# Nikhil-Doye/voice-enabled-browser-automation

Measured on AMD Instinct MI355X. Metric: voice-to-intent p50 latency (ms) + ASR RTF; 10s utterance; Llama-3-8B brain, lower is better.
Workload: dtype bf16; 1 GPU; model=whisper-tiny + llama3-8b, global_batch=1, parallelism=dp1, budget_chars=512, hipgraph=True

## Files before the change

### csrc/bindings.cpp

```cpp
#include <mutex>
#include <torch/extension.h>
#include <ATen/hip/impl/HIPStreamMasqueradingAsCUDA.h>
#include <c10/core/DeviceGuard.h>

#include "kernels/vwa_kernels.h"

namespace {

using at::Tensor;

hipStream_t cur_stream(const Tensor& t) {
  return c10::hip::getCurrentHIPStreamMasqueradingAsCUDA(t.device().index()).stream();
}

const uint16_t* bfp(const Tensor& t) { return reinterpret_cast<const uint16_t*>(t.data_ptr()); }
uint16_t* bfp_mut(const Tensor& t) { return reinterpret_cast<uint16_t*>(t.data_ptr()); }
const uint16_t* bfp_opt(const c10::optional<Tensor>& t) { return t.has_value() ? bfp(*t) : nullptr; }

void check_bf16(const Tensor& t, const char* name) {
  TORCH_CHECK(t.is_cuda(), name, " must be a GPU tensor");
  TORCH_CHECK(t.scalar_type() == at::kBFloat16, name, " must be bf16");
}
void check_contig_rows(const Tensor& t, const char* name) {
  TORCH_CHECK(t.dim() == 2, name, " must be 2-D");
// ... 513 lines not shown
  p.ldr = (int)h.stride(0);
}

DecodeAttnParams decode_params(const Tensor& q, const Tensor& k, const Tensor& v, const Tensor& table,
                               int64_t block_size, int64_t sb, int64_t sh, int64_t stok, const Tensor& ctx_lens,
                               const Tensor& seq_ids, int64_t n_q_heads, int64_t n_kv_heads, int64_t head_dim,
                               double scale, int64_t n_splits, const Tensor& part_o, const Tensor& part_ml,
                               const Tensor& counters, const Tensor& out);

std::tuple<Tensor, int64_t> chain_make(Tensor h, Tensor att, Tensor act, Tensor w_o, Tensor w_gu, Tensor w_down,
                                       double eps, c10::optional<Tensor> w_qkv, int64_t n_q_heads, int64_t n_kv_heads,
                                       int64_t head_dim, c10::optional<Tensor> positions, c10::optional<Tensor> slots,
                                       c10::optional<Tensor> rope, c10::optional<Tensor> q_out,
                                       c10::optional<Tensor> k_cache, c10::optional<Tensor> v_cache, Tensor bar,
                                       Tensor work, c10::optional<Tensor> ts, int64_t bar_mode,
                                       c10::optional<Tensor> a_q, c10::optional<Tensor> a_k, c10::optional<Tensor> a_v,
                                       c10::optional<Tensor> a_table, int64_t a_block_size, int64_t a_sb, int64_t a_sh,
                                       int64_t a_st, c10::optional<Tensor> a_ctx, c10::optional<Tensor> a_seq,
                                       double a_scale, int64_t a_n_splits, c10::optional<Tensor> a_part_o,
                                       c10::optional<Tensor> a_part_ml, c10::optional<Tensor> a_counters,
                                       bool w_tiled, c10::optional<Tensor> a_row_table,
                                       c10::optional<Tensor> s_o, c10::optional<Tensor> s_gu,
                                       c10::optional<Tensor> s_down, c10::optional<Tensor> s_qkv, int64_t tp_ar,
                                       c10::optional<Tensor> a_plan, int64_t a_plan_mode) {
  c10::DeviceGuard g(h.device());
  const int64_t M = h.size(0);
  TORCH_CHECK(att.size(0) == M && act.size(0) == M, "row counts differ");
  TORCH_CHECK(act.size(1) * 2 == w_gu.size(0) && w_gu.size(0) % 32 == 0, "act must be [M, gate_up rows / 2]");
  TORCH_CHECK(w_down.size(1) == act.size(1) && w_down.size(0) == h.size(1) && w_o.size(0) == h.size(1),
              "down / o_proj shapes");
  TORCH_CHECK(bar.is_cuda() && bar.scalar_type() == at::kInt && bar.numel() >= 384 && bar.is_contiguous() &&
                  (reinterpret_cast<uintptr_t>(bar.data_ptr()) & 127) == 0,
              "bar must be a 128-byte aligned int32[>=384] on the GPU");
  ChainParams cp{};
  TORCH_CHECK(s_o.has_value() == s_gu.has_value() && s_o.has_value() == s_down.has_value() &&
                  (!w_qkv.has_value() || s_qkv.has_value() == s_o.has_value()),
              "fp8 chain: every phase's weight needs its scales");
  TORCH_CHECK(!s_o.has_value() || w_tiled, "fp8 chain: tiled fp8 weights only");
  cp.ph[0].p = base_params(att, w_o, c10::nullopt, false, eps, s_o, w_tiled);
  cp.ph[0].epi = 1;
  set_resid(cp.ph[0].p, h);
  cp.ph[1].p = base_params(h, w_gu, c10::nullopt, true, eps, s_gu, w_tiled);
  cp.ph[1].epi = 2;
  check_bf16(act, "act");
  TORCH_CHECK(act.stride(1) == 1, "act rows must be contiguous");
  cp.ph[1].p.Y = act.data_ptr();
  cp.ph[1].p.ldy = (int)act.stride(0);
// ... 46 lines not shown
    cp.attn = decode_params(*a_q, *a_k, *a_v, *a_table, a_block_size, a_sb, a_sh, a_st, *a_ctx, *a_seq, n_q_heads,
                            n_kv_heads, head_dim, a_scale, a_n_splits, *a_part_o, *a_part_ml, *a_counters, att);
    TORCH_CHECK(a_n_splits > 1, "attention phase: the in-launch chunk merge needs n_splits > 1");
    cp.attn_g = (int)(n_q_heads / n_kv_heads);
    TORCH_CHECK(a_row_table.has_value(), "attention phase: a_row_table (per-row block tables) is required");
    TORCH_CHECK(a_block_size == 16, "attention phase: 16-token KV blocks (mq_attention.h FINE addressing)");
    {
      const Tensor& rtab = *a_row_table;
      TORCH_CHECK(rtab.is_cuda() && rtab.scalar_type() == at::kInt && rtab.dim() == 2 && rtab.is_contiguous() &&
                      rtab.size(0) >= M && rtab.size(1) <= 128 && rtab.size(1) % 2 == 0,
                  "a_row_table must be int32 [>= rows, <= 128 (even)] contiguous");
      cp.attn.row_table = rtab.data_ptr<int>();
      cp.attn.rt_stride = (int)rtab.size(1);
    }
    if (a_plan_mode) {
      TORCH_CHECK(a_plan_mode == 1 || a_plan_mode == 2, "a_plan_mode: 1 write, 2 read");
      TORCH_CHECK(a_plan.has_value() && a_plan->is_cuda() && a_plan->scalar_type() == at::kInt && a_plan->is_contiguous() &&
                      a_plan->numel() >= (int64_t)chain_grid(h.device().index()) * 16,
                  "a_plan must be int32 [>= grid * 16] on the GPU");
      cp.attn.plan = a_plan->data_ptr<int>();
      cp.attn.plan_mode = (int)a_plan_mode;
    }
  }
  const int lds = vwa_chain_prepare(&cp, chain_grid(h.device().index()));
  if (lds < 0) return {torch::empty({0}, torch::dtype(torch::kUInt8).device(h.device())), 0};
  Tensor host = torch::empty({(int64_t)sizeof(ChainParams)}, torch::dtype(torch::kUInt8));
  std::memcpy(host.data_ptr(), &cp, sizeof(ChainParams));
  return {host.to(h.device()), (int64_t)lds | (cp.n >= 3 && cp.ph[2].xg ? (int64_t)1 << 24 : 0) |
                                    (cp.d_nt2 ? (int64_t)1 << 27 : 0) |
                                    (s_o.has_value() ? (int64_t)1 << 25 : 0) | (cp.o_nt2 ? (int64_t)1 << 26 : 0)};
}

std::tuple<Tensor, int64_t> chain_make_seq(int64_t seq, std::vector<Tensor> X, std::vector<Tensor> W,
                                           std::vector<c10::optional<Tensor>> bias,
                                           std::vector<c10::optional<Tensor>> ln_c, std::vector<Tensor> Y,
                                           std::vector<int64_t> epi, double eps, int64_t n_heads, int64_t head_dim,
                                           c10::optional<Tensor> positions, c10::optional<Tensor> slots,
                                           c10::optional<Tensor> k_cache, c10::optional<Tensor> v_cache, Tensor bar,
                                           Tensor work, int64_t bar_mode, bool w_tiled) {
  const size_t n = X.size();
  TORCH_CHECK(n >= 2 && n <= (size_t)kChainMaxPhases && W.size() == n && bias.size() == n && ln_c.size() == n &&
                  Y.size() == n && epi.size() == n,
              "chain_make_seq: one X/W/bias/ln_c/Y/epi per phase");
  TORCH_CHECK(seq == 1 || seq == 2, "chain_make_seq: seq 1 (Whisper tail) or 2 (Whisper middle)");
  c10::DeviceGuard g(X[0].device());
  TORCH_CHECK(bar.is_cuda() && bar.scalar_type() == at::kInt && bar.numel() >= 384 && bar.is_contiguous() &&
                  (reinterpret_cast<uintptr_t>(bar.data_ptr()) & 127) == 0,
              "bar must be a 128-byte aligned int32[>=384] on the GPU");
// ... 700 lines not shown
  m.def("ar_destroy", &ar_destroy);
  m.doc() = "MI355X (gfx950) HIP kernels for the voice-web-agent inference engine";
  m.def("skinny_gemm", &skinny_gemm, py::arg("x"), py::arg("w"), py::arg("bias"), py::arg("y"), py::arg("epi"),
        py::arg("fuse_rms"), py::arg("eps"), py::arg("residual"), py::arg("w_scale") = py::none(),
        py::arg("ln_c") = py::none(), py::arg("w_tiled") = false, py::arg("col_mask") = py::none(),
        py::arg("col_mask_off") = 0, py::arg("mask_rows") = 1);
  m.def("skinny_gemm_swiglu", &skinny_gemm_swiglu, py::arg("x"), py::arg("w_gu"), py::arg("bias"), py::arg("h"),
        py::arg("fuse_rms"), py::arg("eps"), py::arg("w_scale") = py::none(), py::arg("w_tiled") = false);
  m.def("skinny_gemm_qkv", &skinny_gemm_qkv, py::arg("x"), py::arg("w_qkv"), py::arg("bias"), py::arg("fuse_rms"),
        py::arg("eps"), py::arg("n_q_heads"), py::arg("n_kv_heads"), py::arg("head_dim"), py::arg("use_rope"),
        py::arg("positions"), py::arg("slots"), py::arg("rope"), py::arg("q_out"), py::arg("k_cache"),
        py::arg("v_cache"), py::arg("w_scale") = py::none(), py::arg("ln_c") = py::none(),
        py::arg("w_tiled") = false);
  m.def("chain_make", &chain_make, py::arg("h"), py::arg("att"), py::arg("act"), py::arg("w_o"), py::arg("w_gu"),
        py::arg("w_down"), py::arg("eps"), py::arg("w_qkv"), py::arg("n_q_heads"), py::arg("n_kv_heads"),
        py::arg("head_dim"), py::arg("positions"), py::arg("slots"), py::arg("rope"), py::arg("q_out"),
        py::arg("k_cache"), py::arg("v_cache"), py::arg("bar"), py::arg("work"), py::arg("ts") = py::none(), py::arg("bar_mode") = 1,
        py::arg("a_q") = py::none(), py::arg("a_k") = py::none(), py::arg("a_v") = py::none(),
        py::arg("a_table") = py::none(), py::arg("a_block_size") = 0, py::arg("a_sb") = 0, py::arg("a_sh") = 0,
        py::arg("a_st") = 0, py::arg("a_ctx") = py::none(), py::arg("a_seq") = py::none(), py::arg("a_scale") = 0.0,
        py::arg("a_n_splits") = 0, py::arg("a_part_o") = py::none(), py::arg("a_part_ml") = py::none(),
        py::arg("a_counters") = py::none(), py::arg("w_tiled") = false, py::arg("a_row_table") = py::none(),
        py::arg("s_o") = py::none(), py::arg("s_gu") = py::none(), py::arg("s_down") = py::none(),
        py::arg("s_qkv") = py::none(), py::arg("tp_ar") = 0, py::arg("a_plan") = py::none(), py::arg("a_plan_mode") = 0);
  m.def("set_small_gemm_bytes", &set_small_gemm_bytes);
  m.def("gemm_set_p8", [](int64_t mode) { vwa_gemm_set_p8((int)mode); });
  m.def("skinny_set_x_skew", [](int64_t skew) { vwa_skinny_set_x_skew((int)skew); });
  m.def("gemm_set_split_fill", [](int64_t pct) { vwa_gemm_set_split_fill((int)pct); });
  m.def("chain_make_seq", &chain_make_seq, py::arg("seq"), py::arg("X"), py::arg("W"), py::arg("bias"),
        py::arg("ln_c"), py::arg("Y"), py::arg("epi"), py::arg("eps"), py::arg("n_heads"), py::arg("head_dim"),
        py::arg("positions"), py::arg("slots"), py::arg("k_cache"), py::arg("v_cache"), py::arg("bar"),
        py::arg("work"), py::arg("bar_mode") = 1, py::arg("w_tiled") = false);
  m.def("chain_run", &chain_run, py::arg("desc"), py::arg("n_phases"), py::arg("lds"), py::arg("like"),
        py::arg("attn_g") = 0, py::arg("seq") = 0, py::arg("n_layers") = 1);
  m.def("alloc_uncached_i32", &alloc_uncached_i32);
  m.def("device_cus", [](Tensor like) { return (int64_t)device_cus(like); });
  m.def("wdec_layers", &wdec_layers, py::arg("flat"), py::arg("n_layers"), py::arg("like"));
  m.def("wdec_run", &wdec_run, py::arg("layers"), py::arg("roles"), py::arg("bufs"), py::arg("ints"), py::arg("eps"),
        py::arg("scale"), py::arg("n_prod"), py::arg("ts") = py::none(), py::arg("opt") = 0, py::arg("lm") = py::none(),
        py::arg("emb") = py::none(), py::arg("smp") = py::none(), py::arg("loop_base_block") = 0);
  m.def("decode_advance", &decode_advance);
  m.def("gemm", &gemm, py::arg("x"), py::arg("w"), py::arg("bias"), py::arg("y"), py::arg("epi"),
        py::arg("rstd") = py::none(), py::arg("residual") = py::none(), py::arg("w_tiled") = false,
        py::arg("ws") = py::none(), py::arg("ss_out") = py::none(), py::arg("ss_zero") = py::none(),
        py::arg("ss_in") = py::none(), py::arg("ss_eps") = 1e-5);
  m.def("row_rstd", &row_rstd);
  m.def("gemm_qkv", &gemm_qkv, py::arg("x"), py::arg("sx"), py::arg("w"), py::arg("sw"), py::arg("bias"),
// ... 29 lines not shown
```

### csrc/kernels/skinny_stream.hip

```cpp
#include "common.h"
#include "vwa_kernels.h"
#include "mq_attention.h"

using namespace vwa;

namespace {

enum Epi { EPI_STORE = 0, EPI_RESID = 1, EPI_SWIGLU = 2, EPI_GELU = 3, EPI_QKV = 4 };

constexpr unsigned kOOB = 0xFFFFFFF0u;

VWA_DEVICE uint4 bload(__amdgpu_buffer_rsrc_t r, unsigned off) {
  u32x4 v = __builtin_amdgcn_raw_buffer_load_b128(r, (int)off, 0, 0);
  return make_uint4(v.x, v.y, v.z, v.w);
}
template <int AUX>
VWA_DEVICE uint4 bload_w(__amdgpu_buffer_rsrc_t r, unsigned off) {
  u32x4 v = __builtin_amdgcn_raw_buffer_load_b128(r, (int)off, 0, AUX);
  return make_uint4(v.x, v.y, v.z, v.w);
}
constexpr unsigned kOOB2 = 0x80000000u;
template <int AUX>
VWA_DEVICE uint4 bload_w_so(__amdgpu_buffer_rsrc_t r, unsigned voff, int soff) {
  u32x4 v = __builtin_amdgcn_raw_buffer_load_b128(r, (int)voff, soff, AUX);
// ... 809 lines not shown
  chain_load<S::NT, S::U, WA, R, XG, F8>(ph.p, ph.nb, wr, it, r);
}

template <int NT, int KS>
VWA_DEVICE void tile_publish(int M, float* red, f32x4 (&acc)[NT], float* slot) {
  const int lane = VWA_TX & 63, w = VWA_TX >> 6;
#pragma unroll
  for (int nt = 0; nt < NT; ++nt)
#pragma unroll
    for (int i = 0; i < 4; ++i) red[((w * NT + nt) * 4 + i) * 64 + lane] = acc[nt][i];
  lds_sync();
  for (int o = VWA_TX; o < M * 16 * NT; o += KS * 64) {
    const int m = o / (16 * NT), nn = o % (16 * NT);
    const int nt = nn >> 4, q = nn & 15;
    const int ln = q + 16 * (m >> 2), i = m & 3;
    float v = 0.f;
#pragma unroll
    for (int ww = 0; ww < KS; ++ww) v += red[((ww * NT + nt) * 4 + i) * 64 + ln];
    st_f32<true>(slot + o, v);
  }
  lds_sync();
}

template <int EPI, int KS, int WA, bool XG = false, bool F8 = false, bool W2 = false, int R>
VWA_DEVICE void chain_phase(const ChainParams& cp, int i, uint4 (&X0)[R], uint4 (&X1)[R], char* smem, int pre2,
                            int hs = 0, int wb0 = 0, int wn = 0, bool has0 = true) {
  constexpr int NT = PhaseShape<EPI, KS, XG, F8, W2>::NT, U = PhaseShape<EPI, KS, XG, F8, W2>::U;
  const ChainPhase& ph = cp.ph[i];
  const SkinnyParams& p = ph.p;
  const int nb = ph.nb, M = p.M, K = p.K;
  const int xstride = K + 8;
  u16* xs = reinterpret_cast<u16*>(smem);
  const int xbytes = XG ? 0 : ((M * xstride * 2) + 15) & ~15;
  float* red = reinterpret_cast<float*>(smem + xbytes);
  float* rs = red + KS * NT * 4 * 64;
  float* mu = rs + 16;
  int* s_flag = reinterpret_cast<int*>(rs + 32);
  const float* mus = p.fuse_rms == 2 ? mu : nullptr;
  const int lane = VWA_TX & 63, w = VWA_TX >> 6;
  const int nl = lane & 15, g = lane >> 4;
  const PhaseRange r = chain_range<KS>(ph, wb0, wn);
  const int first_tile = r.u0 / nb;
  const bool xdma = cp.xdma != 0, stager = xdma && w == KS - 1 && !XG;
  auto pst = [&](int k) {
    const int slot = k < 8 ? 22 + 8 * i + k : -1;
    if (cp.ts && VWA_TX == 0 && slot >= 0) *gp(cp.ts + blockIdx.x * kTsStride + slot) = __builtin_amdgcn_s_memrealtime();
  };
  pst(0);
  if constexpr (XG) {
    chain_load_x<U>(p, nb, X0, 0, r);
    if (pre2) chain_load_x<U>(p, nb, X1, 1, r);
  }
  const int k8 = K / 8;
  const __amdgpu_buffer_rsrc_t rx =
      __builtin_amdgcn_make_buffer_rsrc(const_cast<u16*>(p.X), (short)0, (int)((size_t)M * p.ldx * 2), 0x00020000);
  if (stager) {
    const int pieces = K / 512;
    for (int m = 0; m < M; ++m)
      for (int j = 0; j < pieces; ++j)
        __builtin_amdgcn_raw_ptr_buffer_load_lds(
            rx, (__attribute__((address_space(3))) void*)(xs + m * xstride + j * 512), 16,
            (unsigned)(((size_t)m * p.ldx + j * 512) * 2 + lane * 16), 0, 0, 16);
    asm volatile("" ::: "memory");
  }
  const bool xw = xdma && cp.xwait;
  if (xdma && cp.xfirst && !xw) lds_sync();
  auto issue_rest = [&]() {
    if (xdma && !stager && !has0) chain_load<NT, U, WA, R, XG, F8>(p, nb, X0, 0, r);
    if (xdma && !stager && (!pre2 || !has0)) chain_load<NT, U, WA, R, XG, F8>(p, nb, X1, 1, r);
  };
  if (!xw) issue_rest();

  EpiPre pre;
  if (r.n_items > 0 && !xw) epi_values<EPI, NT, true>(p, first_tile, VWA_TX, pre);
  if (stager && xw) {
    asm volatile("s_waitcnt vmcnt(0)" ::: "memory");
  } else if (stager) {
    int nw = 0;
    if (hs < 1) {
      chain_load<NT, U, WA, R, XG, F8>(p, nb, X0, 0, r);
      ++nw;
    }
    if (hs < 2) {
      chain_load<NT, U, WA, R, XG, F8>(p, nb, X1, 1, r);
      ++nw;
    }
    if constexpr (R == 16) {
      if (nw == 2) asm volatile("s_waitcnt vmcnt(32)" ::: "memory");
      else if (nw == 1) asm volatile("s_waitcnt vmcnt(16)" ::: "memory");
      else asm volatile("s_waitcnt vmcnt(0)" ::: "memory");
    } else {
      static_assert(R == 8, "item sizes: 16 or 8 loads");
      if (nw == 2) asm volatile("s_waitcnt vmcnt(16)" ::: "memory");
      else if (nw == 1) asm volatile("s_waitcnt vmcnt(8)" ::: "memory");
      else asm volatile("s_waitcnt vmcnt(0)" ::: "memory");
    }
  } else if (!xdma && !XG) {
    for (int c = VWA_TX; c < M * k8; c += KS * 64) {
      const int m = c / k8, kk = c % k8;
      const u32x4 v = __builtin_amdgcn_raw_buffer_load_b128(rx, (int)(((size_t)m * p.ldx + kk * 8) * 2), 0, 16);
      *reinterpret_cast<uint4*>(xs + m * xstride + kk * 8) = make_uint4(v.x, v.y, v.z, v.w);
    }
  }
  lds_sync();
  pst(1);
  auto issue_xw = [&]() {
    issue_rest();
    if (stager) {
      if (hs < 1) chain_load<NT, U, WA, R, XG, F8>(p, nb, X0, 0, r);
      if (hs < 2) chain_load<NT, U, WA, R, XG, F8>(p, nb, X1, 1, r);
    }
    if (r.n_items > 0) epi_values<EPI, NT, true>(p, first_tile, VWA_TX, pre);
  };
  if (xw && !cp.xw_late) issue_xw();
  for (int m = w; m < 16; m += KS) {
    float sc = 1.f, mean = 0.f;
    if (p.fuse_rms && m < M && !XG) {
      float s = 0.f, s1 = 0.f;
      for (int kk = lane; kk < k8; kk += 64) {
        float f[8];
        unpack8(*reinterpret_cast<const uint4*>(xs + m * xstride + kk * 8), f);
#pragma unroll
        for (int j = 0; j < 8; ++j) {
          s += f[j] * f[j];
          s1 += f[j];
        }
      }
// ... 173 lines not shown
  const int tx = VWA_TX, lane = tx & 63, w = tx >> 6;
  const __amdgpu_buffer_rsrc_t rk = __builtin_amdgcn_make_buffer_rsrc(const_cast<u16*>(a.kv.k), (short)0, 0x7FFFFFF0, 0x00020000);
  const __amdgpu_buffer_rsrc_t rv = __builtin_amdgcn_make_buffer_rsrc(const_cast<u16*>(a.kv.v), (short)0, 0x7FFFFFF0, 0x00020000);
  const __amdgpu_buffer_rsrc_t rt = __builtin_amdgcn_make_buffer_rsrc(const_cast<int*>(a.row_table), (short)0,
                                                                     (r0 + 1) * a.rt_stride * 4, 0x00020000);
  auto* dst = (__attribute__((address_space(3))) void*)(lds + w * kMqStep * 256);
  int blk[4];
#pragma unroll
  for (int i = 0; i < 4; ++i) {
    const int q = w * 64 + lane + 512 * i, key = kbeg + q / 16;
    blk[i] = (int)__builtin_amdgcn_raw_buffer_load_b32(rt, q < nk * 16 ? (r0 * a.rt_stride + key / 16) * 4 : 0x7FFFFFF0,
                                                       0, 0);
  }
#pragma unroll
  for (int i = 0; i < 4; ++i) {
    const int q = w * 64 + lane + 512 * i, key = kbeg + q / 16;
    if (512 * i + w * 64 >= nk * 16) break;
    const long long e = (long long)blk[i] * a.kv.stride_block + (long long)kvh * a.kv.stride_head +
                        (long long)(key & 15) * a.kv.stride_tok;
    const unsigned off = q < nk * 16 ? (unsigned)(e * 2 + (q & 15) * 16) : 0x7FFFFFF0u;
    __builtin_amdgcn_raw_ptr_buffer_load_lds(rk, dst, 16, off, 0, 0, 0);
    __builtin_amdgcn_raw_ptr_buffer_load_lds(rv, dst, 16, off, 0, 0, 0);
  }
}

template <int KS, int SEQ, int NPH, int AG, int WA, bool XG2 = false, bool F8 = false, bool O2 = false, bool D2 = false,
          bool MULTI = false>
__global__ __launch_bounds__(KS * 64) void chain_kernel(const ChainParams* __restrict__ cpp, int n_layers) {
  extern __shared__ __attribute__((aligned(16))) char smem[];
  static_assert(!MULTI || (SEQ == 0 && NPH == 4 && AG > 0 && !XG2), "multi-layer launch: Llama tails with attention");
  const int nwg = (int)gridDim.x;
  unsigned long long* bar = reinterpret_cast<unsigned long long*>(cpp->bar);
  unsigned long long bar_next = chain_base(bar, nwg, cpp->bar_mode);
  const bool tpr = cpp->tp.world > 1;
  const int e0 = tpr ? __hip_atomic_load(gp(cpp->tp.epoch), __ATOMIC_RELAXED, __HIP_MEMORY_SCOPE_AGENT) : 0;
  unsigned long long qkv_base[8] = {};
  const bool qsig = MULTI && cpp->qkv_flags && cpp->bar_mode == 2 && cpp->ph[3].nb == 1 &&
                    cpp->ph[3].p.n_kv_heads <= 8 && cpp->attn_flag;
  if constexpr (MULTI) {
    if (qsig && VWA_TX < 64) {
      const unsigned long long tpg = (unsigned long long)qkv_tiles_per_group(cpp->ph[3].p);
      for (int g = 0; g < cpp->ph[3].p.n_kv_heads; ++g) {
        const unsigned long long v = __hip_atomic_load(gp(&bar[kBarQkv + kBarQkvStride * g]), __ATOMIC_RELAXED, __HIP_MEMORY_SCOPE_AGENT);
        qkv_base[g] = v / tpg * tpg;
      }
    }
  }
  bool pf_prev = false, pf_next = false;
  for (int li = 0; li < (MULTI ? n_layers : 1); ++li) {
  pf_prev = pf_next;
  pf_next = false;
  const ChainParams& cp = cpp[li];
  static_assert(sizeof(ChainParams) <= 25 * 64, "descriptor warm-up covers 25 lines");
  {
    unsigned junk;
    asm("s_load_dword %0, %1, 0x0\n\t""s_load_dword %0, %1, 0x40\n\t""s_load_dword %0, %1, 0x80\n\t""s_load_dword %0, %1, 0xc0\n\t"
        "s_load_dword %0, %1, 0x100\n\t""s_load_dword %0, %1, 0x140\n\t""s_load_dword %0, %1, 0x180\n\t""s_load_dword %0, %1, 0x1c0\n\t"
        "s_load_dword %0, %1, 0x200\n\t""s_load_dword %0, %1, 0x240\n\t""s_load_dword %0, %1, 0x280\n\t""s_load_dword %0, %1, 0x2c0\n\t"
        "s_load_dword %0, %1, 0x300\n\t""s_load_dword %0, %1, 0x340\n\t""s_load_dword %0, %1, 0x380\n\t""s_load_dword %0, %1, 0x3c0\n\t"
        "s_load_dword %0, %1, 0x400\n\t""s_load_dword %0, %1, 0x440\n\t""s_load_dword %0, %1, 0x480\n\t""s_load_dword %0, %1, 0x4c0\n\t""s_load_dword %0, %1, 0x500\n\t"
        "s_load_dword %0, %1, 0x540\n\t""s_load_dword %0, %1, 0x580\n\t""s_load_dword %0, %1, 0x5c0\n\t""s_load_dword %0, %1, 0x600\n\t"
        "s_waitcnt lgkmcnt(0)"
        : "=&s"(junk)
        : "s"(cpp + li));
    if (junk == 0x9e3779b9u) __builtin_amdgcn_s_sleep(1);
  }
  uint4 A[ChainShape<KS, F8>::R] = {}, B[ChainShape<KS, F8>::R] = {};
  unsigned long long gen;
  const int er = e0 + 2 * li;
  int nts = 0;
  auto stamp = [&]() {
    if (cp.ts && VWA_TX == 0) *gp(cp.ts + blockIdx.x * kTsStride + nts) = __builtin_amdgcn_s_memrealtime();
// ... 145 lines not shown
   }
  }
  if constexpr (MULTI) {
    if (li + 1 < n_layers) {
      if (qsig) qkv_signal<KS>(cp.ph[3], bar);
      else gen = chain_arrive(bar, nwg, cp.bar_mode, bar_next);
      const DecodeAttnParams& na = cpp[li + 1].attn;
      int st = 3, ev = 0;
      if (cpp[li + 1].attn_flag && na.plan_mode == 2) {
        const __amdgpu_buffer_rsrc_t r_pl =
            __builtin_amdgcn_make_buffer_rsrc(na.plan, (short)0, ((int)blockIdx.x + 1) * 64, 0x00020000);
        ev = (int)__builtin_amdgcn_raw_buffer_load_b32(r_pl, ((int)blockIdx.x * 16 + (VWA_TX & 15)) * 4, 0, 16);
        st = __builtin_amdgcn_readlane(ev, 10) == na.rows ? __builtin_amdgcn_readlane(ev, 2) : 3;
      }
      if (st != 0 && st != 2) {
        if (st == 1 && cp.kv_prefetch) {
          kv_prefetch(na, ev, reinterpret_cast<unsigned char*>(smem));
          pf_next = true;
        }
        if (!qsig) {
          chain_wait(bar, gen, cp.bar_mode);
        } else {
          const int kvh = __builtin_amdgcn_readlane(ev, 3);
          const unsigned long long add = (unsigned long long)qkv_tiles_per_group(cp.ph[3].p) * (unsigned long long)(li + 1);
          if (st == 1) qkv_wait(bar, qkv_base, add, kvh, kvh + 1);
          else qkv_wait(bar, qkv_base, add, 0, cp.ph[3].p.n_kv_heads);
        }
      }
    }
  }
  }
}

}

extern "C" int vwa_chain_prepare(ChainParams* cp, int grid) {
  constexpr int KS = 8;
  constexpr int R = ChainShape<KS>::R;
  if (cp->n < 2 || cp->n > kChainMaxPhases || grid < 1) return -10;
  static const int kSeq[3][kChainMaxPhases] = {{EPI_RESID, EPI_SWIGLU, EPI_RESID, EPI_QKV},
                                               {EPI_RESID, EPI_GELU, EPI_RESID, EPI_QKV},
                                               {EPI_RESID, EPI_STORE, -1, -1}};
  if (cp->seq < 0 || cp->seq > 2 || (cp->seq == 2 ? cp->n != 2 : cp->n < (cp->seq == 0 ? 2 : 3))) return -10;
  if (cp->seq == 0 && cp->n == 2) return -10;
  size_t lds = 0;
  for (int i = 0; i < cp->n; ++i) {
    ChainPhase& ph = cp->ph[i];
// ... 193 lines not shown
```

### csrc/kernels/vwa_kernels.h

```cpp
#pragma once
#include <hip/hip_runtime.h>
#include <stdint.h>

struct SkinnyParams {
  const uint16_t* X; int ldx;
  const uint16_t* W;
  int M, N, K;
  const uint16_t* bias;
  int fuse_rms; float eps;
  void* Y; int ldy; int y_f32;
  const uint16_t* R; int ldr;
  int n_q_heads, n_kv_heads, head_dim, use_rope;
  const int* positions;
  const int64_t* slots;
  const float* rope;
  uint16_t* q_out; int ldq;
  uint16_t* k_cache; uint16_t* v_cache;
  int block_size;
  int64_t cache_stride_block, cache_stride_head, cache_stride_tok;
  const float* w_scale;
  int w_first;
  const float* ln_c;
  int w_tiled;
  const uint32_t* col_mask; int col_mask_ld; int col_mask_rows;
// ... 54 lines not shown
  int max_tiles;
  unsigned long long* ts;
  DecodeAttnParams attn;
  int attn_g;
  int lds_item;
  int lds_item_waves;
  int lds_item_req;
  int lds_item2;
  int lds_item2_waves;
  int lds_item2_req;
  int attn_flag;
  int pre_mask;
  int pre_waves;
  int xfirst;
  int xwait;
  int xw_late;
  int poll_free;
  int o_nt2;
  int d_nt2;
  int kv_prefetch;
  int qkv_flags;
  int attn_pre;
  ChainTP tp;
};

struct GemmParams {
  const uint16_t* X; int ldx;
  const uint16_t* W; int w_tiled;
  int M, N, K;
  void* Y; int ldy; int y_f32;
  const uint16_t* bias;
  const uint16_t* R; int ldr;
  const float* rstd;
  float* ws; int splits; int kg_per_split;
  const float* sx; const float* sw;
  int nbatch; int64_t bsx, bsy, bsr;
  int cus; int64_t ws_cap;
  int n_q_heads, n_kv_heads, head_dim, use_rope;
  const int* positions; const int64_t* slots; const float* rope;
  uint16_t* q_out; int ldq; uint16_t* k_cache; uint16_t* v_cache; int block_size;
  int64_t cache_sb, cache_sh, cache_st;
  unsigned long long* ss_out; unsigned long long* ss_zero; int ss_zero_n; const unsigned long long* ss_in;
  float ss_eps;
};

struct FlashAttnParams {
// ... 104 lines not shown
```

### voice_enabled_browser_automation_amd/models/llama.py

```python
from __future__ import annotations

import weakref
from dataclasses import dataclass
from typing import List, Optional

import torch

from .. import ops
from ..parallel.tp import TPContext
from .config import LlamaConfig


@dataclass
class LlamaLayerWeights:
    qkv: torch.Tensor
    o: torch.Tensor
    gu: torch.Tensor
    down: torch.Tensor


def _randn(gen: torch.Generator, shape, std: float, device, dtype) -> torch.Tensor:
    t = torch.empty(shape, device=device, dtype=torch.float32)
    t.normal_(0.0, std, generator=gen)
    return t.to(dtype)
# ... 165 lines not shown
                and not getattr(self, "_chain_gated", False)
                and ops.env_flag("VWA_CHAIN") and ops.native_available())

    def _chain_any(self, M: int) -> bool:
        return self._chain_ok(M)

    def disable_chain(self) -> None:
        self._chain_disabled = True
        self.reset_chains()

    def enable_chain(self) -> None:
        if self.tp.size > 1:
            return
        for t in (getattr(self, "_chain_bar", None), getattr(self, "_chain_work", None)):
            if t is not None:
                t.zero_()
        self._chain_disabled = False
        self.reset_chains()

    def reset_chains(self) -> None:
        self._chains = weakref.WeakKeyDictionary()

    def chain_descs(self):
        return [v for d in getattr(self, "_chains", {}).values() for k, v in d.items() if k[0] != "multi"]

    def _chain_desc(self, bufs, kv, M: int, li: int):
        if not isinstance(getattr(self, "_chains", None), weakref.WeakKeyDictionary):
            self.reset_chains()
        cache = self._chains.setdefault(bufs, {})
        key = (M, li, kv.k[li].data_ptr(), kv.v[li].data_ptr(), bufs.max_ctx)
        if key in cache:
            return cache[key]
        if getattr(self, "_chain_bar", None) is None:
            self._chain_bar, self._chain_bar_mode, self._chain_work = ops.chain_buffers(self.device)
        L = self.layers[li]
        nxt = li + 1 < len(self.layers)
        N = self.layers[li + 1] if nxt else None
        attn = (M <= 4 and self.hd == 128 and self.nq // self.nkv in (4, 8) and ops.env_flag("VWA_CHAIN_ATTN")
                and ops.decode_n_splits(bufs.max_ctx) > 1 and getattr(bufs, "rt_cols", 0) > 0
                and kv.k[li].shape[2] == 16)
        a = {}
        if attn:
            lay = ops.KVLayout.paged(kv.k[li], kv.v[li], bufs.block_table)
            a = dict(a_q=bufs.q[:M], a_k=lay.k, a_v=lay.v, a_table=lay.table, a_block_size=lay.block_size,
                     a_sb=lay.sb, a_sh=lay.sh, a_st=lay.st, a_ctx=bufs.ctx_lens, a_seq=bufs.seq_ids,
                     a_scale=self.scale, a_n_splits=ops.decode_n_splits(bufs.max_ctx), a_part_o=bufs.part_o,
                     a_part_ml=bufs.part_ml, a_counters=bufs.attn_cnt, a_row_table=bufs.row_table)
            if ops.env_flag("VWA_CHAIN_PLAN"):
                if getattr(bufs, "attn_plan", None) is None:
                    bufs.attn_plan = torch.zeros(1024 * 16, dtype=torch.int32, device=self.device)
                a.update(a_plan=bufs.attn_plan, a_plan_mode=1 if li == 0 else 2)
        f8 = isinstance(L.o, ops.FP8Weight)
        tiled = f8 or isinstance(L.o, ops.TiledWeight)
        wsel = (lambda w: w.w8) if f8 else (lambda w: w.t) if tiled else (lambda w: w)
        sc = {}
        if f8:
            sc = dict(s_o=L.o.scale, s_gu=L.gu.scale, s_down=L.down.scale, s_qkv=N.qkv.scale if nxt else None)
        def make(a):
            return ops.ext().chain_make(
                bufs.hidden[:M], bufs.attn[:M], bufs.act[:M], wsel(L.o), wsel(L.gu), wsel(L.down), self.cfg.rms_eps,
                wsel(N.qkv) if nxt else None, self.nq, self.nkv, self.hd,
                bufs.positions if nxt else None, bufs.slots if nxt else None, self.rope if nxt else None,
                bufs.q[:M] if nxt else None, kv.k[li + 1] if nxt else None, kv.v[li + 1] if nxt else None,
                self._chain_bar, self._chain_work, None, self._chain_bar_mode, **a, w_tiled=tiled, **sc,
                tp_ar=self.tp.custom_ar.state if self.tp.size > 1 else 0)

        desc, lds = make(a)
        if not desc.numel() and attn:
            attn = False
            desc, lds = make({})
        cache[key] = (desc, 4 if nxt else 3, lds, self.nq // self.nkv if attn else 0) if desc.numel() else None
        return cache[key]

    def _chain_multi(self, bufs, kv, M: int):
        n = len(self.layers)
        if n < 3 or not ops.env_flag("VWA_CHAIN_MULTI") or self.tp.size > 1 and not ops.env_flag("VWA_CHAIN_TP"):
            return None
        cache = self._chains.setdefault(bufs, {}) if isinstance(getattr(self, "_chains", None), weakref.WeakKeyDictionary) else None
        key = ("multi", M, tuple(kv.k[li].data_ptr() for li in range(n)),
               tuple(kv.v[li].data_ptr() for li in range(n)), bufs.max_ctx)
        if cache is not None and key in cache:
            return cache[key]
        ds = [self._chain_desc(bufs, kv, M, li) for li in range(n)]
        ok = (all(d is not None and d[3] > 0 for d in ds) and all(d[1] == 4 for d in ds[:-1]) and ds[-1][1] == 3
              and len({(d[2], d[3]) for d in ds}) == 1)
        lds = ds[0][2] if ok else 0
        ok = ok and not (lds >> 24) & 1 and ((lds >> 25) & 1) != ((lds >> 26) & 1)
        out = (torch.cat([d[0] for d in ds]), lds, ds[0][3], n) if ok else None
        self._chains.setdefault(bufs, {})[key] = out
        return out

    def chain_error_word(self):
        return ops.chain_error_word(getattr(self, "_chain_bar", None))

    def chain_error(self) -> bool:
        bar = getattr(self, "_chain_bar", None)
        return bool(bar is not None and int(bar.view(torch.int64)[160].item()) != 0)

    def forward(self, bufs, M: int, kv, *, prefill_seq: Optional[int] = None, q_offset: int = 0,
                logits_rows: Optional[slice] = None, n_sel: Optional[int] = None, head: bool = True) -> torch.Tensor:
        cfg = self.cfg
        h = bufs.hidden[:M]
        ops.embedding(bufs.tokens, self.embed, out=h, rows=M, vocab_start=self.v_start)
        if self.tp.size > 1:
            self.tp.all_reduce(h)
        qbuf = bufs.q[:M] if M <= bufs.q.shape[0] else torch.empty((M, self.nq * self.hd), dtype=self.dtype,
                                                                      device=self.device)
        chain = prefill_seq is None and self._chain_ok(M)
        pf_slices = None
        if (prefill_seq is not None and q_offset >= M and M <= 256 and self.device.type == "cuda"
                and ops.env_flag("VWA_PREFILL_DECODE_ATTN")):
            i32 = dict(dtype=torch.int32, device=self.device)
            pf_ctx = torch.arange(q_offset + 1, q_offset + M + 1, **i32)
            pf_sid = torch.full((M,), prefill_seq, **i32)
            pf_slices = [(i, min(M, i + 64)) for i in range(0, M, 64)]
            pf_out = torch.empty((M, self.nq * self.hd), dtype=self.dtype, device=self.device)
        ss = self._rms_stats(M) if not chain else None
        multi = self._chain_multi(bufs, kv, M) if chain else None
        for li, L in enumerate(self.layers):
            kc, vc = kv.k[li], kv.v[li]
            if multi is not None and li < multi[3]:
                if li == 0:
                    ops.qkv_rope_write(h, L.qkv, None, fuse_rms=True, eps=cfg.rms_eps, n_q_heads=self.nq,
                                       n_kv_heads=self.nkv, head_dim=self.hd, rope=self.rope, positions=bufs.positions,
                                       slots=bufs.slots, q_out=qbuf, k_cache=kc, v_cache=vc)
                    ops.ext().chain_run(multi[0], 4, multi[1], h, multi[2], 0, multi[3])
                continue
            if chain and li > 0:
                q = qbuf
            else:
                q = ops.qkv_rope_write(h, L.qkv, None, fuse_rms=True, eps=cfg.rms_eps, n_q_heads=self.nq,
                                       n_kv_heads=self.nkv, head_dim=self.hd, rope=self.rope,
                                       positions=bufs.positions, slots=bufs.slots, q_out=qbuf, k_cache=kc, v_cache=vc,
                                       ss_in=ss[1] if ss is not None and li > 0 else None)
            d = self._chain_desc(bufs, kv, M, li) if chain else None
            if d is not None:
                if not d[3]:
                    ops.decode_attention(q, ops.KVLayout.paged(kc, vc, bufs.block_table), bufs.ctx_lens,
                                         bufs.seq_ids, n_q_heads=self.nq, n_kv_heads=self.nkv, head_dim=self.hd,
                                         scale=self.scale, max_ctx=bufs.max_ctx, out=bufs.attn[:M],
                                         part_o=bufs.part_o, part_ml=bufs.part_ml, counters=bufs.attn_cnt,
                                         shared=getattr(bufs, "shared", None))
                ops.ext().chain_run(d[0], d[1], d[2], h, d[3])
                continue
            chain = False
            if prefill_seq is None:
                attn = bufs.attn[:M]
                fl = getattr(bufs, "flash", None)
                if fl is not None:
# ... 71 lines not shown
```

### voice_enabled_browser_automation_amd/utils/env.py

```python
from __future__ import annotations

import os
from typing import Any, Optional

from pydantic import BaseModel, Field


def _parse_env_file(path: str) -> dict:
    out = {}
    try:
        with open(path, "r", encoding="utf-8") as fh:
            for line in fh:
                line = line.strip()
                if not line or line.startswith("#") or "=" not in line:
                    continue
                k, v = line.split("=", 1)
                k = k.strip()
                if k.startswith("export "):
                    k = k[7:].strip()
                v = v.strip()
                if len(v) >= 2 and v[0] == v[-1] and v[0] in "\"'":
                    v = v[1:-1]
                out[k] = v
    except OSError:
# ... 75 lines not shown
    VWA_KV_GB: str = Field("0", description="paged-KV budget in GB, 0: per max_seqs x max_len, auto: HBM plan")
    VWA_ROW_BUCKETS: str = Field("1,2,4,8,12,16,32,48,64", description="decode row buckets of the captured graphs")
    VWA_SHARED_ATTN: bool = Field(True, description="decode attention reads a shared prompt prefix once per row group")
    VWA_PREFILL_FLASH: bool = Field(True, description="batched admission prefill through one causal flash launch")
    VWA_RMS_HANDOFF: bool = Field(True, description="> 16-row steps: residual GEMMs hand the next RMSNorm its row statistics (no row_rstd launches)")
    VWA_FP8_A16_ROWS: int = Field(64, description="fp8 weights: rows up to which the > 16-row GEMM runs W8A16 (no activation quantisation)")
    VWA_PREFILL_DECODE_ATTN: bool = Field(True, description="cached-prefix prompt suffix through the decode attention")
    VWA_TILED_WEIGHTS: bool = Field(True, description="keep projection weights only in the MFMA-tiled layout")
    VWA_MASKED_HEAD: bool = Field(True, description="LM head computes only the vocab tiles the grammar admits")
    VWA_SPIN_WAIT: bool = Field(True, description="wait for a step's tokens by polling the pinned readback")
    VWA_ZERO_COPY: bool = Field(True, description="grammar masks written straight into pinned step memory")
    VWA_ASR_DEVICE_LOOP: bool = Field(True, description="single-session Whisper greedy loop resident on the GPU")
    VWA_CHAIN: bool = Field(True, description="chained Llama decode layer (skinny_stream.hip chain_kernel)")
    VWA_CHAIN_ATTN: bool = Field(True, description="decode attention as the chained launch's phase 0")
    VWA_CHAIN_MAX_ROWS: int = Field(4, description="rows per step the chained launch takes")
    VWA_CHAIN_TP: bool = Field(True, description="chained launch with in-launch TP all-reduce rounds")
    VWA_CHAIN_RETRY: bool = Field(True, description="re-arm the chain after a barrier-timeout fallback")
    VWA_CHAIN_ASR: bool = Field(False, description="chained Whisper decoder launches (measured slower; off)")
    VWA_WDEC_OPT: int = Field(0, description="diagnostic: schedule option bits of the persistent Whisper decoder (whisper_dec.hip kOpt*; 0 = the measured defaults)")
    VWA_ASR_PERSIST: bool = Field(True, description="one-row Whisper decode steps (every width, tiny .. large) as ONE persistent launch: embedding, every decoder layer, LM head and, in the device loop, argmax + advance (csrc/kernels/whisper_dec.hip); needs every CU free: off when the GPU is shared with a persistent brain launch")
    VWA_CHAIN_GRID_DIV: Optional[str] = Field(None, description="chained launch on CUs / k workgroups (shared GPU)")
    VWA_CHAIN_PLAN: bool = Field(True, description="chained attention: layer 0 writes the step's work plan, layers 1.. read it")
    VWA_CHAIN_MULTI: bool = Field(True, description="chained decode: all layers in ONE launch (skinny_stream.hip chain_kernel MULTI)")
    VWA_CHAIN_BAR_MODE: int = Field(2, description="chained launches' grid barrier: 2 two-level tickets + scalar polls (default), 4 no-return arrivals + polled sum of the 8 group counters")
    VWA_CHAIN_SCHED: Optional[str] = Field(None, description="DIAGNOSTIC: chained schedule override name=value,...")
    VWA_GEMM_QKV: bool = Field(True, description="> 16-row QKV: rotary + KV write in the tiled GEMM epilogue")
    VWA_GEMM_P8: Optional[str] = Field(None, description="DIAGNOSTIC: 256x256 8-phase GEMM eligibility override")
    VWA_GEMM_SPLIT_FILL: Optional[str] = Field(None, description="DIAGNOSTIC: split-K fill target (% of CUs)")
    VWA_SKINNY_X_SKEW: Optional[str] = Field(None, description="DIAGNOSTIC: LDS X-row skew of the streaming GEMM")
    VWA_ATTN_IMPL: Optional[str] = Field(None, description="DIAGNOSTIC: decode attention implementation")
    VWA_KERNEL_SO: Optional[str] = Field(None, description="DIAGNOSTIC: another build of the kernel library (A/B)")
    VWA_STRICT_NATIVE: bool = Field(False, description="vendor-library fallbacks in the op layer raise (tests, bench)")
    VWA_BENCH_CONCURRENT: int = Field(0, description="bench.py --full: concurrent sessions (0: the headline only)")
    VWA_FORCE_BUILD: bool = Field(False, description="__graft_entry__.build(): recompile every source")
    VWA_HIPCC_EXTRA: str = Field("", description="extra hipcc flags (experiments)")

    @classmethod
    def from_env(cls) -> "Settings":
        return cls(**{name: knob(name) for name in cls.model_fields})


_TRUE = ("1", "true", "yes", "on")


def _parse(name: str, raw: str) -> Any:
    ann = Settings.model_fields[name].annotation
# ... 26 lines not shown
```

Measured before the change: 236.8 ms.

## Fold embedding gather and layer-0 QKV into the multi-layer chained decode launch

Adds an entry phase to the persistent multi-layer chain kernel. It gathers the step's token embedding rows straight from the embedding table into LDS, writes them back to the hidden buffer, and runs layer 0's QKV/rope/KV-write phase before a grid barrier, so the separate embedding and qkv_rope_write launches per decode step go away. This targets launch and inter-kernel gaps for bf16, single-rank, small-row decode. The cost is an extra grid barrier plus scalar-cache warming at kernel entry, and a more complex barrier-count accounting (li0 offset) that could be fragile.

```diff
diff --git a/csrc/bindings.cpp b/csrc/bindings.cpp
--- a/csrc/bindings.cpp
+++ b/csrc/bindings.cpp
@@ -559,7 +559,8 @@
                                        bool w_tiled, c10::optional<Tensor> a_row_table,
                                        c10::optional<Tensor> s_o, c10::optional<Tensor> s_gu,
                                        c10::optional<Tensor> s_down, c10::optional<Tensor> s_qkv, int64_t tp_ar,
-                                       c10::optional<Tensor> a_plan, int64_t a_plan_mode) {
+                                       c10::optional<Tensor> a_plan, int64_t a_plan_mode,
+                                       c10::optional<Tensor> e_ids, c10::optional<Tensor> e_table) {
   c10::DeviceGuard g(h.device());
   const int64_t M = h.size(0);
   TORCH_CHECK(att.size(0) == M && act.size(0) == M, "row counts differ");
@@ -652,8 +653,24 @@
       cp.attn.plan_mode = (int)a_plan_mode;
     }
   }
+  if (e_ids.has_value()) {
+    TORCH_CHECK(e_table.has_value() && w_qkv.has_value() && a_q.has_value() && !s_o.has_value() && !tp_ar && M <= 4,
+                "entry descriptor: the bf16 QKV phase of a one-rank attention chain of <= 4 rows");
+    TORCH_CHECK(e_ids->is_cuda() && e_ids->scalar_type() == at::kInt && e_ids->is_contiguous() && e_ids->numel() >= 4 &&
+                    (reinterpret_cast<uintptr_t>(e_ids->data_ptr()) & 3) == 0,
+                "e_ids must be int32 [>= 4] on the GPU");
+    check_bf16(*e_table, "e_table");
+    TORCH_CHECK(e_table->is_cuda() && e_table->dim() == 2 && e_table->is_contiguous() && e_table->size(1) == h.size(1) &&
+                    h.stride(1) == 1 && (size_t)e_table->numel() * 2 < 0x7FFFFFF0ull,
+                "e_table must be bf16 [rows, hidden] contiguous and below 2 GB");
+    cp.entry = 1;
+    cp.e_ids = e_ids->data_ptr<int>();
+    cp.e_table = bfp(*e_table);
+    cp.e_rows = (int)e_table->size(0);
+  }
   const int lds = vwa_chain_prepare(&cp, chain_grid(h.device().index()));
   if (lds < 0) return {torch::empty({0}, torch::dtype(torch::kUInt8).device(h.device())), 0};
+  if (cp.entry && cp.ph[3].nb != 1) return {torch::empty({0}, torch::dtype(torch::kUInt8).device(h.device())), 0};
   Tensor host = torch::empty({(int64_t)sizeof(ChainParams)}, torch::dtype(torch::kUInt8));
   std::memcpy(host.data_ptr(), &cp, sizeof(ChainParams));
   return {host.to(h.device()), (int64_t)lds | (cp.n >= 3 && cp.ph[2].xg ? (int64_t)1 << 24 : 0) |
@@ -1400,7 +1417,8 @@
         py::arg("a_n_splits") = 0, py::arg("a_part_o") = py::none(), py::arg("a_part_ml") = py::none(),
         py::arg("a_counters") = py::none(), py::arg("w_tiled") = false, py::arg("a_row_table") = py::none(),
         py::arg("s_o") = py::none(), py::arg("s_gu") = py::none(), py::arg("s_down") = py::none(),
-        py::arg("s_qkv") = py::none(), py::arg("tp_ar") = 0, py::arg("a_plan") = py::none(), py::arg("a_plan_mode") = 0);
+        py::arg("s_qkv") = py::none(), py::arg("tp_ar") = 0, py::arg("a_plan") = py::none(), py::arg("a_plan_mode") = 0,
+        py::arg("e_ids") = py::none(), py::arg("e_table") = py::none());
   m.def("set_small_gemm_bytes", &set_small_gemm_bytes);
   m.def("gemm_set_p8", [](int64_t mode) { vwa_gemm_set_p8((int)mode); });
   m.def("skinny_set_x_skew", [](int64_t skew) { vwa_skinny_set_x_skew((int)skew); });
diff --git a/csrc/kernels/skinny_stream.hip b/csrc/kernels/skinny_stream.hip
--- a/csrc/kernels/skinny_stream.hip
+++ b/csrc/kernels/skinny_stream.hip
@@ -855,7 +855,7 @@
   lds_sync();
 }
 
-template <int EPI, int KS, int WA, bool XG = false, bool F8 = false, bool W2 = false, int R>
+template <int EPI, int KS, int WA, bool XG = false, bool F8 = false, bool W2 = false, bool ENT = false, int R>
 VWA_DEVICE void chain_phase(const ChainParams& cp, int i, uint4 (&X0)[R], uint4 (&X1)[R], char* smem, int pre2,
                             int hs = 0, int wb0 = 0, int wn = 0, bool has0 = true) {
   constexpr int NT = PhaseShape<EPI, KS, XG, F8, W2>::NT, U = PhaseShape<EPI, KS, XG, F8, W2>::U;
@@ -885,15 +885,41 @@
     if (pre2) chain_load_x<U>(p, nb, X1, 1, r);
   }
   const int k8 = K / 8;
-  const __amdgpu_buffer_rsrc_t rx =
-      __builtin_amdgcn_make_buffer_rsrc(const_cast<u16*>(p.X), (short)0, (int)((size_t)M * p.ldx * 2), 0x00020000);
+  static_assert(!ENT || (EPI == EPI_QKV && !XG && !F8), "entry: the bf16 QKV phase");
+  constexpr bool ent = ENT;
+  int eid0 = 0, eid1 = 0, eid2 = 0, eid3 = 0;
+  if (ent)
+    asm("s_load_dword %0, %4, 0x0\n\t"
+        "s_load_dword %1, %4, 0x4\n\t"
+        "s_load_dword %2, %4, 0x8\n\t"
+        "s_load_dword %3, %4, 0xc\n\t"
+        "s_waitcnt lgkmcnt(0)"
+        : "=&s"(eid0), "=&s"(eid1), "=&s"(eid2), "=&s"(eid3)
+        : "s"(cp.e_ids));
+  const __amdgpu_buffer_rsrc_t rx = __builtin_amdgcn_make_buffer_rsrc(
+      const_cast<u16*>(ent ? cp.e_table : p.X), (short)0,
+      (int)(ent ? (size_t)cp.e_rows * K * 2 : (size_t)M * p.ldx * 2), 0x00020000);
+  auto xrow_off = [&](int m) -> unsigned {
+    if (ent) {
+      const int id = m == 0 ? eid0 : m == 1 ? eid1 : m == 2 ? eid2 : eid3;
+      return id >= 0 && id < cp.e_rows ? (unsigned)id * (unsigned)K * 2u : kOOB2;
+    }
+    return (unsigned)((size_t)m * p.ldx * 2);
+  };
   if (stager) {
     const int pieces = K / 512;
-    for (int m = 0; m < M; ++m)
+    for (int m = 0; m < M; ++m) {
+      const unsigned ro = xrow_off(m);
+      if (ent && ro == kOOB2) {
+        for (int j = 0; j < pieces; ++j)
+          *reinterpret_cast<uint4*>(xs + m * xstride + j * 512 + lane * 8) = make_uint4(0, 0, 0, 0);
+        continue;
+      }
       for (int j = 0; j < pieces; ++j)
         __builtin_amdgcn_raw_ptr_buffer_load_lds(
             rx, (__attribute__((address_space(3))) void*)(xs + m * xstride + j * 512), 16,
-            (unsigned)(((size_t)m * p.ldx + j * 512) * 2 + lane * 16), 0, 0, 16);
+            ro + (unsigned)(j * 1024 + lane * 16), 0, 0, 16);
+    }
     asm volatile("" ::: "memory");
   }
   const bool xw = xdma && cp.xwait;
@@ -931,11 +957,21 @@
   } else if (!xdma && !XG) {
     for (int c = VWA_TX; c < M * k8; c += KS * 64) {
       const int m = c / k8, kk = c % k8;
-      const u32x4 v = __builtin_amdgcn_raw_buffer_load_b128(rx, (int)(((size_t)m * p.ldx + kk * 8) * 2), 0, 16);
+      const unsigned ro = xrow_off(m);
+      const u32x4 v = __builtin_amdgcn_raw_buffer_load_b128(rx, (int)(ent && ro == kOOB2 ? kOOB2 : ro + kk * 16), 0, 16);
       *reinterpret_cast<uint4*>(xs + m * xstride + kk * 8) = make_uint4(v.x, v.y, v.z, v.w);
     }
   }
   lds_sync();
+  if (ent) {
+    const __amdgpu_buffer_rsrc_t rh =
+        __builtin_amdgcn_make_buffer_rsrc(const_cast<u16*>(p.X), (short)0, (int)((size_t)M * p.ldx * 2), 0x00020000);
+    for (int c = (int)blockIdx.x * KS * 64 + VWA_TX; c < M * k8; c += (int)gridDim.x * KS * 64) {
+      const int m = c / k8, kk = c % k8;
+      const uint4 v = *reinterpret_cast<const uint4*>(xs + m * xstride + kk * 8);
+      __builtin_amdgcn_raw_buffer_store_b128(u32x4{v.x, v.y, v.z, v.w}, rh, (int)(((size_t)m * p.ldx + kk * 8) * 2), 0, 16);
+    }
+  }
   pst(1);
   auto issue_xw = [&]() {
     issue_rest();
@@ -1155,6 +1191,20 @@
     __builtin_amdgcn_raw_ptr_buffer_load_lds(rk, dst, 16, off, 0, 0, 0);
     __builtin_amdgcn_raw_ptr_buffer_load_lds(rv, dst, 16, off, 0, 0, 0);
   }
+}
+
+VWA_DEVICE void chain_warm(const ChainParams* d) {
+  unsigned junk;
+  asm("s_load_dword %0, %1, 0x0\n\t""s_load_dword %0, %1, 0x40\n\t""s_load_dword %0, %1, 0x80\n\t""s_load_dword %0, %1, 0xc0\n\t"
+      "s_load_dword %0, %1, 0x100\n\t""s_load_dword %0, %1, 0x140\n\t""s_load_dword %0, %1, 0x180\n\t""s_load_dword %0, %1, 0x1c0\n\t"
+      "s_load_dword %0, %1, 0x200\n\t""s_load_dword %0, %1, 0x240\n\t""s_load_dword %0, %1, 0x280\n\t""s_load_dword %0, %1, 0x2c0\n\t"
+      "s_load_dword %0, %1, 0x300\n\t""s_load_dword %0, %1, 0x340\n\t""s_load_dword %0, %1, 0x380\n\t""s_load_dword %0, %1, 0x3c0\n\t"
+      "s_load_dword %0, %1, 0x400\n\t""s_load_dword %0, %1, 0x440\n\t""s_load_dword %0, %1, 0x480\n\t""s_load_dword %0, %1, 0x4c0\n\t""s_load_dword %0, %1, 0x500\n\t"
+      "s_load_dword %0, %1, 0x540\n\t""s_load_dword %0, %1, 0x580\n\t""s_load_dword %0, %1, 0x5c0\n\t""s_load_dword %0, %1, 0x600\n\t"
+      "s_waitcnt lgkmcnt(0)"
+      : "=&s"(junk)
+      : "s"(d));
+  if (junk == 0x9e3779b9u) __builtin_amdgcn_s_sleep(1);
 }
 
 template <int KS, int SEQ, int NPH, int AG, int WA, bool XG2 = false, bool F8 = false, bool O2 = false, bool D2 = false,
@@ -1179,8 +1229,26 @@
       }
     }
   }
+  int li0 = 0;
+  if constexpr (MULTI && !F8) {
+    if (cpp->entry) {
+      const ChainParams& cp = cpp[0];
+      chain_warm(cpp);
+      constexpr int E3 = SeqEpi<SEQ, 3>::value;
+      uint4 A[ChainShape<KS, F8>::R] = {}, B[ChainShape<KS, F8>::R] = {};
+      const int wv = (int)(VWA_TX >> 6);
+      const bool stg = cp.xdma && wv == KS - 1;
+      const bool prew = (cp.pre_waves == 0 || wv < cp.pre_waves) && !(cp.poll_free && wv == 0);
+      const int pre3 = ((cp.pre_mask >> 3) & 1) ? 1 : cp.xdma ? 0 : cp.pre2;
+      if (!stg && prew) chain_issue_first<E3, KS, WA, false, F8>(cp.ph[3], A, B, pre3);
+      chain_phase<E3, KS, WA, false, F8, false, true>(cp, 3, A, B, smem, pre3, 0, 0, 0, prew);
+      const unsigned long long gen = chain_arrive(bar, nwg, cp.bar_mode, bar_next);
+      chain_wait(bar, gen, cp.bar_mode);
+      li0 = 1;
+    }
+  }
   bool pf_prev = false, pf_next = false;
-  for (int li = 0; li < (MULTI ? n_layers : 1); ++li) {
+  for (int li = li0; li < (MULTI ? n_layers : 1); ++li) {
   pf_prev = pf_next;
   pf_next = false;
   const ChainParams& cp = cpp[li];
@@ -1372,7 +1440,7 @@
           chain_wait(bar, gen, cp.bar_mode);
         } else {
           const int kvh = __builtin_amdgcn_readlane(ev, 3);
-          const unsigned long long add = (unsigned long long)qkv_tiles_per_group(cp.ph[3].p) * (unsigned long long)(li + 1);
+          const unsigned long long add = (unsigned long long)qkv_tiles_per_group(cp.ph[3].p) * (unsigned long long)(li + 1 - li0);
           if (st == 1) qkv_wait(bar, qkv_base, add, kvh, kvh + 1);
           else qkv_wait(bar, qkv_base, add, 0, cp.ph[3].p.n_kv_heads);
         }
diff --git a/csrc/kernels/vwa_kernels.h b/csrc/kernels/vwa_kernels.h
--- a/csrc/kernels/vwa_kernels.h
+++ b/csrc/kernels/vwa_kernels.h
@@ -100,6 +100,10 @@
   int qkv_flags;
   int attn_pre;
   ChainTP tp;
+  int entry;
+  int e_rows;
+  const int* e_ids;
+  const uint16_t* e_table;
 };
 
 struct GemmParams {
diff --git a/voice_enabled_browser_automation_amd/models/llama.py b/voice_enabled_browser_automation_amd/models/llama.py
--- a/voice_enabled_browser_automation_amd/models/llama.py
+++ b/voice_enabled_browser_automation_amd/models/llama.py
@@ -211,20 +211,21 @@
         self._chains = weakref.WeakKeyDictionary()
 
     def chain_descs(self):
-        return [v for d in getattr(self, "_chains", {}).values() for k, v in d.items() if k[0] != "multi"]
-
-    def _chain_desc(self, bufs, kv, M: int, li: int):
+        return [v for d in getattr(self, "_chains", {}).values() for k, v in d.items() if k[0] not in ("multi", "entry")]
+
+    def _chain_desc(self, bufs, kv, M: int, li: int, entry: bool = False):
         if not isinstance(getattr(self, "_chains", None), weakref.WeakKeyDictionary):
             self.reset_chains()
         cache = self._chains.setdefault(bufs, {})
-        key = (M, li, kv.k[li].data_ptr(), kv.v[li].data_ptr(), bufs.max_ctx)
+        key = ("entry" if entry else M, M if entry else li, kv.k[li].data_ptr(), kv.v[li].data_ptr(), bufs.max_ctx)
         if key in cache:
             return cache[key]
         if getattr(self, "_chain_bar", None) is None:
             self._chain_bar, self._chain_bar_mode, self._chain_work = ops.chain_buffers(self.device)
         L = self.layers[li]
-        nxt = li + 1 < len(self.layers)
-        N = self.layers[li + 1] if nxt else None
+        nxt = entry or li + 1 < len(self.layers)
+        nl = li if entry else li + 1
+        N = self.layers[nl] if nxt else None
         attn = (M <= 4 and self.hd == 128 and self.nq // self.nkv in (4, 8) and ops.env_flag("VWA_CHAIN_ATTN")
                 and ops.decode_n_splits(bufs.max_ctx) > 1 and getattr(bufs, "rt_cols", 0) > 0
                 and kv.k[li].shape[2] == 16)
@@ -250,12 +251,16 @@
                 bufs.hidden[:M], bufs.attn[:M], bufs.act[:M], wsel(L.o), wsel(L.gu), wsel(L.down), self.cfg.rms_eps,
                 wsel(N.qkv) if nxt else None, self.nq, self.nkv, self.hd,
                 bufs.positions if nxt else None, bufs.slots if nxt else None, self.rope if nxt else None,
-                bufs.q[:M] if nxt else None, kv.k[li + 1] if nxt else None, kv.v[li + 1] if nxt else None,
+                bufs.q[:M] if nxt else None, kv.k[nl] if nxt else None, kv.v[nl] if nxt else None,
                 self._chain_bar, self._chain_work, None, self._chain_bar_mode, **a, w_tiled=tiled, **sc,
-                tp_ar=self.tp.custom_ar.state if self.tp.size > 1 else 0)
-
+                tp_ar=self.tp.custom_ar.state if self.tp.size > 1 else 0,
+                **(dict(e_ids=bufs.tokens, e_table=self.embed) if entry else {}))
+
+        if entry and not attn:
+            cache[key] = None
+            return None
         desc, lds = make(a)
-        if not desc.numel() and attn:
+        if not desc.numel() and attn and not entry:
             attn = False
             desc, lds = make({})
         cache[key] = (desc, 4 if nxt else 3, lds, self.nq // self.nkv if attn else 0) if desc.numel() else None
@@ -275,7 +280,16 @@
               and len({(d[2], d[3]) for d in ds}) == 1)
         lds = ds[0][2] if ok else 0
         ok = ok and not (lds >> 24) & 1 and ((lds >> 25) & 1) != ((lds >> 26) & 1)
-        out = (torch.cat([d[0] for d in ds]), lds, ds[0][3], n) if ok else None
+        front = None
+        if (ok and self.tp.size == 1 and self.wdtype == "bf16" and self.v_start == 0
+                and bufs.tokens.dtype == torch.int32 and bufs.tokens.numel() >= 4
+                and self.embed.dtype == torch.bfloat16 and self.embed.is_contiguous()
+                and self.embed.numel() * 2 < 0x7FFFFFF0 and ops.env_flag("VWA_STEP_ONE_LAUNCH")):
+            front = self._chain_desc(bufs, kv, M, 0, entry=True)
+            if front is not None and (front[1], front[2], front[3]) != (4, lds, ds[0][3]):
+                front = None
+        descs = ([front[0]] if front is not None else []) + [d[0] for d in ds]
+        out = (torch.cat(descs), lds, ds[0][3], n, front is not None) if ok else None
         self._chains.setdefault(bufs, {})[key] = out
         return out
 
@@ -290,12 +304,15 @@
                 logits_rows: Optional[slice] = None, n_sel: Optional[int] = None, head: bool = True) -> torch.Tensor:
         cfg = self.cfg
         h = bufs.hidden[:M]
-        ops.embedding(bufs.tokens, self.embed, out=h, rows=M, vocab_start=self.v_start)
-        if self.tp.size > 1:
-            self.tp.all_reduce(h)
+        chain = prefill_seq is None and self._chain_ok(M)
+        multi = self._chain_multi(bufs, kv, M) if chain else None
+        front = multi is not None and multi[4]
+        if not front:
+            ops.embedding(bufs.tokens, self.embed, out=h, rows=M, vocab_start=self.v_start)
+            if self.tp.size > 1:
+                self.tp.all_reduce(h)
         qbuf = bufs.q[:M] if M <= bufs.q.shape[0] else torch.empty((M, self.nq * self.hd), dtype=self.dtype,
                                                                       device=self.device)
-        chain = prefill_seq is None and self._chain_ok(M)
         pf_slices = None
         if (prefill_seq is not None and q_offset >= M and M <= 256 and self.device.type == "cuda"
                 and ops.env_flag("VWA_PREFILL_DECODE_ATTN")):
@@ -305,15 +322,16 @@
             pf_slices = [(i, min(M, i + 64)) for i in range(0, M, 64)]
             pf_out = torch.empty((M, self.nq * self.hd), dtype=self.dtype, device=self.device)
         ss = self._rms_stats(M) if not chain else None
-        multi = self._chain_multi(bufs, kv, M) if chain else None
         for li, L in enumerate(self.layers):
             kc, vc = kv.k[li], kv.v[li]
             if multi is not None and li < multi[3]:
                 if li == 0:
-                    ops.qkv_rope_write(h, L.qkv, None, fuse_rms=True, eps=cfg.rms_eps, n_q_heads=self.nq,
-                                       n_kv_heads=self.nkv, head_dim=self.hd, rope=self.rope, positions=bufs.positions,
-                                       slots=bufs.slots, q_out=qbuf, k_cache=kc, v_cache=vc)
-                    ops.ext().chain_run(multi[0], 4, multi[1], h, multi[2], 0, multi[3])
+                    if not front:
+                        ops.qkv_rope_write(h, L.qkv, None, fuse_rms=True, eps=cfg.rms_eps, n_q_heads=self.nq,
+                                           n_kv_heads=self.nkv, head_dim=self.hd, rope=self.rope,
+                                           positions=bufs.positions, slots=bufs.slots, q_out=qbuf, k_cache=kc,
+                                           v_cache=vc)
+                    ops.ext().chain_run(multi[0], 4, multi[1], h, multi[2], 0, multi[3] + (1 if front else 0))
                 continue
             if chain and li > 0:
                 q = qbuf
diff --git a/voice_enabled_browser_automation_amd/utils/env.py b/voice_enabled_browser_automation_amd/utils/env.py
--- a/voice_enabled_browser_automation_amd/utils/env.py
+++ b/voice_enabled_browser_automation_amd/utils/env.py
@@ -121,6 +121,7 @@
     VWA_CHAIN_GRID_DIV: Optional[str] = Field(None, description="chained launch on CUs / k workgroups (shared GPU)")
     VWA_CHAIN_PLAN: bool = Field(True, description="chained attention: layer 0 writes the step's work plan, layers 1.. read it")
     VWA_CHAIN_MULTI: bool = Field(True, description="chained decode: all layers in ONE launch (skinny_stream.hip chain_kernel MULTI)")
+    VWA_STEP_ONE_LAUNCH: bool = Field(True, description="multi-layer chained launch also gathers the step's embedding rows and runs layer 0's QKV phase (no embedding / qkv_rope_write launches; bf16, one rank, <= 4 rows)")
     VWA_CHAIN_BAR_MODE: int = Field(2, description="chained launches' grid barrier: 2 two-level tickets + scalar polls (default), 4 no-return arrivals + polled sum of the 8 group counters")
     VWA_CHAIN_SCHED: Optional[str] = Field(None, description="DIAGNOSTIC: chained schedule override name=value,...")
     VWA_GEMM_QKV: bool = Field(True, description="> 16-row QKV: rotary + KV write in the tiled GEMM epilogue")
```

Measured after the change: 237.5 ms. About the same (+0.3%).
